# ctu-mrs/space_filling_forest_star

Hardware: AMD Instinct MI355X
Metric: accepted node expansions/sec + collision checks/sec, dense_3D 6-DoF (higher is better)
Workload: dtype f64

## Files before the change

space_filling_forest_star_amd/csrc/devforest.hip:

```cpp
#include <hip/hip_runtime.h>
#include <stdint.h>
#include <stdlib.h>
#include "kernels.h"
#include "sff_geom.h"
#include "kernels_dev.h"

namespace sffk {

using namespace sffg;

__device__ __forceinline__ int record_words_dev(int nbcap) { return 6 + 4 * nbcap; }

__device__ __forceinline__ int lemire_pick(unsigned long long word, unsigned long long range) {
  const unsigned long long lo = word * range;
  const unsigned long long hi = __umul64hi(word, range);
  if (lo < range) {
    const unsigned long long thr = (0ULL - range) % range;
    if (lo < thr) return -1;
  }
  return (int)hi;
}

__device__ __forceinline__ int32_t* frontier_now(const DevForestView& f) { return f.ctrl->front_sel ? f.frontier2 : f.frontier; }
__device__ __forceinline__ int32_t* act_now(const DevForestView& f) { return f.ctrl->act_sel ? f.act_slot2 : f.act_slot; }
// ... 159 lines not shown
#define KC_WLO 2
#define KC_WHI 3
#define KC_POSTED 4
#define KC_OWN 5
#define KC_CNT 6
#define KC_DEP 12
#define KC_EVN 13

__device__ __forceinline__ unsigned long long kc_load(const unsigned long long* p) {
  return __hip_atomic_load(p, __ATOMIC_RELAXED, __HIP_MEMORY_SCOPE_AGENT);
}
__device__ __forceinline__ void kc_publish(unsigned long long* p, unsigned seq, unsigned v) {
  __hip_atomic_store(p, ((unsigned long long)seq << 32) | (unsigned long long)v, __ATOMIC_RELAXED, __HIP_MEMORY_SCOPE_AGENT);
}
__device__ __forceinline__ unsigned kc_wait(const unsigned long long* p, unsigned seq, int32_t* fault) {
  for (int spin = 0; spin < KC_SPIN_LIMIT; ++spin) {
    const unsigned long long v = kc_load(p);
    if ((unsigned)(v >> 32) == seq) return (unsigned)v;
    __builtin_amdgcn_s_sleep(1);
  }
  atomicOr(fault, 1);
  return 0u;
}
__device__ __forceinline__ unsigned long long kc_block_sum(unsigned long long v, unsigned long long* slot) {
  for (int off = 32; off > 0; off >>= 1) v += __shfl_xor(v, off);
  __syncthreads();
  if (threadIdx.x == 0) *slot = 0ULL;
  __syncthreads();
  if ((threadIdx.x & 63) == 0 && v) atomicAdd(slot, v);
  __syncthreads();
  return *slot;
}

__device__ __forceinline__ void kc_block_sum8(unsigned long long* v, unsigned long long* slots, int from) {
  for (int q = from; q < 8; ++q)
    for (int off = 32; off > 0; off >>= 1) v[q] += __shfl_xor(v[q], off);
  __syncthreads();
  if (threadIdx.x < 8) slots[threadIdx.x] = 0ULL;
  __syncthreads();
  if ((threadIdx.x & 63) == 0)
    for (int q = from; q < 8; ++q) if (v[q]) atomicAdd(&slots[q], v[q]);
  __syncthreads();
  for (int q = from; q < 8; ++q) v[q] = slots[q];
}

__global__ __launch_bounds__(1024) void k_commit(ResolveArgs A, int n_bound) {
  __shared__ int s_state[64], s_dk[64], s_dep[64];
  __shared__ unsigned long long s_cnt[64][6];
  __shared__ unsigned long long s_sum;
  __shared__ unsigned long long s_wa, s_we, s_c6[7];
  __shared__ int s_ev_total;
  __shared__ unsigned long long s_tot[8];
  __shared__ DevCtrl K;
  const DevForestView& f = A.f;
  DevCtrl* c = f.ctrl;
  const int b = blockIdx.x;
  const int grp = threadIdx.x >> 4, gl = threadIdx.x & 15, lane = threadIdx.x & 63;
  const int i = b * 64 + grp;
  const bool inb = i < n_bound;
  const size_t s0 = (size_t)i * A.stride;
  const bool inl = inb && A.in_lim[i] != 0;
  const int flags = inb ? A.rec_flags[i] : 0;
  int nnb = inb ? A.rec_nnb[i] : 0;
  const bool pose_hit = inb && A.pose_hit[i] != 0;
  int fh = 0x7fffffff, ns = 0, nb = 0, meta = 0;
  if (inb) {
    fh = A.first_hit[s0 + gl]; ns = A.seg_ns[s0 + gl];
    if (gl > 0) { nb = A.rec_nb[(size_t)i * A.nbcap + gl - 1]; meta = A.rec_meta[(size_t)i * A.nbcap + gl - 1]; }
  }
  const int halt = c->halt, n = c->n_act;
  if (halt || n == 0) {
    if (b == 0 && threadIdx.x == 0) {
      c->app_n = 0;
      if (A.star) { A.S.hdr[0] = 0; A.S.hdr[1] = 1; A.S.hdr[2] = 0; A.S.hdr[4] = 0; }
    }
    return;
  }
  if (b == 0 && f.ord.hist)
    for (int r = threadIdx.x; r < f.ord.n_sub; r += 1024) (c->act_sel ? f.ord.cnt[0] : f.ord.cnt[1])[r * SFFK_ORD_CNT_STRIDE] = 0;
  if (b * 64 >= n) return;
  const int nwg = (n + 63) >> 6;
  const bool last = b == nwg - 1;
  const unsigned seq = (unsigned)f.commit_seq[0] + 1u;
  const int seq30 = (int)(seq & 0x3fffffffu);
  const int Tb = f.temp_base, N0 = c->N0, nb0 = c->n_borders;
  const unsigned long long stamp_hi = (c->epoch + 1ULL) << 32;
  unsigned long long* pub = f.wg_pub + (size_t)b * SFFK_PUB_WORDS;
  unsigned long long tk[6];
  const bool clk = last && f.profile;
  tk[0] = clk ? wall_clock64() : 0ULL;
  unsigned long long* trace = (f.kc_trace && (int)c->rounds == f.kc_trace_round && threadIdx.x == 0) ? f.kc_trace + 8 * (size_t)b : nullptr;
#define KC_TRACE(k) do { if (trace) trace[k] = wall_clock64(); } while (0)
  KC_TRACE(0);
  int work_items = 0;
  if (last) {
    for (int w = threadIdx.x; w < (int)(sizeof(DevCtrl) / 4); w += 1024)
      reinterpret_cast<int32_t*>(&K)[w] = reinterpret_cast<const int32_t*>(c)[w];
    work_items = A.round_ctrl[2];
  }

  auto calls_of = [](int fh, int ns) -> unsigned long long {
    return fh != 0x7fffffff ? (unsigned long long)fh : (unsigned long long)ns;
  };
  const int gsh = lane & 48;
  auto gballot = [&](bool p) -> unsigned { return (unsigned)((__ballot(p) >> gsh) & 0xffffULL); };
  auto gsum = [&](unsigned long long v) -> unsigned long long {
    for (int off = 8; off > 0; off >>= 1) v += __shfl_xor(v, off);
    return v;
  };
  unsigned long long cnt[6] = {0, 0, 0, 0, 0, 0};
  int st = 1, code = SFFK_REJECTED, dk = 0, was_dep = 0;
  const bool live = i < n;
  bool pending = false;
  if (nnb > 15) nnb = 15;
  const bool have = gl <= nnb;
  if (!have) { fh = 0x7fffffff; ns = 0; nb = 0; meta = 0; }
  const bool is_nb = have && gl > 0;
  const bool mate = is_nb && nb >= Tb;
  const bool same = (meta & 1) != 0;
  const bool fr = fh == 0x7fffffff;
  const unsigned long long my_calls = calls_of(fh, ns);
  const unsigned stops = gballot(is_nb && (mate || !same || fr));
  const unsigned mates = gballot(mate), sames = gballot(same), frees = gballot(fr);
  const bool goal_mode = f.goal_id >= 0;
  const unsigned goals = gballot(goal_mode && is_nb && nb == f.goal_id);
  bool count_end = true;
  if (live) {
    if (!inl) code = SFFK_OUTSIDE;
    else if (flags & 2) { if (gl == 0) { atomicOr(A.fault_pending, 1); atomicAdd(A.fault_pending + 1, 1); KC_FAULT_SETTLE(); } }
    else if ((flags & 3) == 1) {
      const bool ovf = gballot(have && fh == 0) != 0;
      const bool mine = A.world <= 1 || i % A.world == A.rank;
      const unsigned long long smp = gsum(have ? (unsigned long long)ns : 0ULL);
      if (mine) { cnt[3] = 1; cnt[4] = 1 + (unsigned long long)nnb; cnt[5] = smp; }
      const int fh0 = __shfl(fh, gsh), ns0 = __shfl(ns, gsh);
      if (ovf) { if (gl == 0) { atomicOr(A.fault_pending, 1); atomicAdd(A.fault_pending + 2, 1); KC_FAULT_SETTLE(); } }
      else {
        cnt[0] = 1;
        if (!pose_hit) {
          cnt[1] = 1;
          cnt[0] += calls_of(fh0, ns0);
          if (fh0 == 0x7fffffff) {
            cnt[2] = (unsigned long long)f.n_trees;
            pending = true;
          }
// ... 197 lines not shown
      ev_pref = (int)kc_block_sum(pe, &s_sum);
    }
    KC_TRACE(6);
    if (own) {
      const int at = nb0 + ev_pref + __popcll(wo & ((1ULL << threadIdx.x) - 1ULL));
      double pn[6], pe6[6], dn;
      int ta;
      const int raw = A.rec_nb[(size_t)e_i * A.nbcap + s_dk[threadIdx.x]];
      if (raw >= Tb) {
        const int j = raw - Tb;
        for (int q = 0; q < 6; ++q) pn[q] = A.newpos[6 * (size_t)j + q];
        dn = A.pdist[j] + f.d_root[A.parent[j]];
        ta = A.st.tree[A.parent[j]];
      } else {
        for (int q = 0; q < 6; ++q) pn[q] = A.st.pos[6 * (size_t)e_nb + q];
        dn = f.d_root[e_nb];
        ta = A.st.tree[e_nb];
      }
      const int tb = A.st.tree[e_ex];
      f.b_n1[at] = e_nb < e_ex ? e_nb : e_ex; f.b_n2[at] = e_nb < e_ex ? e_ex : e_nb;
      f.b_ta[at] = ta < tb ? ta : tb; f.b_tb[at] = ta < tb ? tb : ta;
      for (int q = 0; q < 6; ++q) pe6[q] = A.st.pos[6 * (size_t)e_ex + q];
      if (A.star) {
        const int e = at - nb0;
        A.S.ev_sample[e] = e_i; A.S.ev_nb[e] = e_nb; A.S.ev_ex[e] = e_ex; A.S.ev_dist[e] = dist6(pn, pe6);
        f.b_dist[at] = 0.0;
      } else
      f.b_dist[at] = dn + f.d_root[e_ex] + dist6(pn, pe6);
      f.pair[(size_t)ta * f.n_trees + tb] = 1;
      f.pair[(size_t)tb * f.n_trees + ta] = 1;
    }
  }
  KC_TRACE(7);
  if (!last) return;
  if (clk) tk[3] = wall_clock64();
  unsigned long long q_end = 0ULL, q_beg = ~0ULL;
  if (f.qclk_sh && threadIdx.x < 64) {
    q_end = f.qclk_sh[threadIdx.x * 16]; q_beg = f.qclk_sh[threadIdx.x * 16 + 1];
    for (int off = 32; off > 0; off >>= 1) {
      const unsigned long long e2 = __shfl_xor(q_end, off), b2 = __shfl_xor(q_beg, off);
      q_end = e2 > q_end ? e2 : q_end; q_beg = b2 < q_beg ? b2 : q_beg;
    }
  }
  unsigned long long tot[8] = {0, 0, 0, 0, 0, 0, 0, 0};
  if ((int)threadIdx.x < b) {
    const unsigned long long* pp = f.wg_pub + (size_t)threadIdx.x * SFFK_PUB_WORDS;
    for (int q = 0; q < 8; ++q) tot[q] = (unsigned)(early[q] >> 32) == seq ? (unsigned)early[q] : kc_wait(pp + KC_CNT + q, seq, f.commit_seq + 6);
  }
  if (threadIdx.x == 1023) s_ev_total = fault_seen;
  kc_block_sum8(tot, s_tot, 0);
  for (int q = 0; q < 7; ++q) tot[q] += s_c6[q];
  tot[7] += (unsigned long long)__popcll(we);
  const int n_acc = acc_pref + __popcll(wa), n_ev = defer ? (int)tot[7] : ev_pref + n_own, n_dep = (int)tot[6];
  const bool faulted = s_ev_total != 0;
  auto roll_back = [&](DevCtrl* k) {
    k->fault = SFFK_FAULT_LISTS;
    k->halt = 1;
    k->round -= 1;
    k->iter = k->iter0;
    k->cursor = k->words_base;
    k->rounds -= 1;
    k->round_nodes -= (unsigned long long)(k->N0 + n);
    k->round_queries -= (unsigned long long)n;
    k->n_act = 0;
    k->app_n = 0;
  };
  if (A.star && !faulted) {
    for (int w = threadIdx.x; w < (int)(sizeof(DevCtrl) / 4); w += 1024)
      reinterpret_cast<int32_t*>(A.S.backup)[w] = reinterpret_cast<const int32_t*>(&K)[w];
    __syncthreads();
    if (threadIdx.x == 0) roll_back(A.S.backup);
  }
  if (threadIdx.x == 0) {
    if (faulted) {
      roll_back(&K);
      *A.fault_pending = 0;
      if (A.star) { A.S.hdr[0] = 0; A.S.hdr[1] = 1; A.S.hdr[2] = 0; A.S.hdr[4] = 0; }
    } else {
      const int fn0 = K.frontier_n, act_cnt = K.act_cnt, act_sel = K.act_sel;
      K.collide_calls += tot[0];
      K.path_free_calls += tot[1];
      K.nn_queries += tot[2];
      K.poses_executed += tot[3];
      K.segments_executed += tot[4];
      K.samples_executed += tot[5];
      K.work_items += (unsigned long long)work_items;
      if (f.qclk_sh) { K.q_t0 = q_beg; K.q_t1 = q_end; }
      if (K.q_t1 > K.q_t0) { K.q_ticks += K.q_t1 - K.q_t0; K.q_launches += 1ULL; }
      K.app_n = n;
      K.app_N0 = N0;
      K.app_fn0 = fn0;
      K.app_act_sel = act_sel;
      K.app_act_cnt = act_cnt;
      K.iter0_app = K.iter0;
      K.n_nodes = N0 + n_acc;
      K.frontier_n = f.prio.n_heaps ? fn0 : fn0 + n_acc;
      K.n_borders = nb0 + n_ev;
      K.app_nb0 = nb0;
      K.n_unsettled += n_dep;
      K.epoch += 1ULL;
      if (A.star) {
        K.nn_queries += (unsigned long long)n_acc;
        A.S.hdr[0] = n_acc; A.S.hdr[1] = 0; A.S.hdr[2] = n_ev; A.S.hdr[3] = nb0; A.S.hdr[4] = 0;
      }
      K.act_sel = act_sel ^ 1;
      K.act_cnt = (n - n_acc) + (act_cnt - n);
      round_begin_scalars(f, &K);
      if (clk) {
        tk[4] = wall_clock64();
        for (int q = 0; q < 4; ++q) K.prof[q] += tk[q + 1] - tk[q];
      }
      K.prof[5] += (unsigned long long)passes;
      K.prof[6] += 1ULL;
      if ((unsigned long long)passes > K.prof[7]) K.prof[7] = (unsigned long long)passes;
    }
    f.commit_seq[0] = (int32_t)seq;
  }
  __syncthreads();
  for (int w = threadIdx.x; w < (int)(sizeof(DevCtrl) / 4); w += 1024)
    reinterpret_cast<int32_t*>(c)[w] = reinterpret_cast<const int32_t*>(&K)[w];
}

__device__ __forceinline__ void append_ord_store(const ResolveArgs& A, int ord_at, int next) {
  if (ord_at >= 0) (A.f.ctrl->app_act_sel ? A.f.ord.lst[0] : A.f.ord.lst[1])[ord_at] = next;
}
__device__ __forceinline__ int append_one(const ResolveArgs& A, int i, int& slot_out, int& ord_at, int part = 0) {
  ord_at = -1;
  const DevForestView& f = A.f;
  const DevCtrl* c = f.ctrl;
  const int n = c->app_n;
  slot_out = -1;
  if (n <= 0) return -1;
  const int act_cnt = c->app_act_cnt;
  const int32_t* act_old = c->app_act_sel ? f.act_slot2 : f.act_slot;
  int32_t* act_new = c->app_act_sel ? f.act_slot : f.act_slot2;
  const bool wave_over = c->n_act == 0 && !c->halt && c->in_wave && !c->use_closed;
  const bool ord_on = f.ord.hist && c->ord_valid;
  auto claim = [&](int e, int slot) {
    const int nd = f.slot_node[slot];
    atomicMin(&f.claim[nd], e);
    f.ulist[e] = nd;
  };
  if (wave_over && i == 0 && part != 1) f.ctrl->claims_done = 1;
  if (i >= n) {
    if (i < act_cnt && part != 1) {
      const int e = (c->act_cnt - (act_cnt - n)) + (i - n), slot = act_old[i];
      act_new[e] = slot;
      if (wave_over) claim(e, slot);
    }
    return -1;
  }
  const unsigned long long w = f.w_acc[i >> 6];
  const int rank = f.acc_pref[i >> 6] + __popcll(w & ((1ULL << (i & 63)) - 1ULL));
// ... 451 lines not shown
```

space_filling_forest_star_amd/csrc/engine.cpp:

```cpp
#include "engine.h"
#include <dlfcn.h>

#include <algorithm>
#include <chrono>
#include <cmath>
#include <cstdlib>
#include <cstring>
#include <limits>

#include "sff_geom.h"

namespace sff {

void hip_check(hipError_t e, const char* what) {
  if (e != hipSuccess) throw HipError{std::string(what) + ": " + hipGetErrorString(e)};
}
#define HIPCHK(x) hip_check((x), #x)

void DevBuf::ensure(size_t bytes) {
  if (bytes <= cap) return;
  size_t want = std::max(bytes, cap * 2);
  want = (want + 255) & ~(size_t)255;
  void* np = nullptr;
  HIPCHK(hipMalloc(&np, want));
// ... 262 lines not shown
  double ms = kernel_ms[kind];
  if (round_timed[kind]) ms += round_ms[kind] * ((double)round_calls[kind] / (double)round_timed[kind]);
  return ms;
}
void Ctx::sync() {
  HIPCHK(hipStreamSynchronize(stream));
  for (auto& t : pending) {
    float ms = 0;
    HIPCHK(hipEventElapsedTime(&ms, t.a, t.b));
    if (t.round) { round_ms[t.kind] += ms; round_timed[t.kind] += 1; }
    else kernel_ms[t.kind] += ms;
    kernel_launches[t.kind] += 1;
    pool.push_back(t.a);
    pool.push_back(t.b);
  }
  pending.clear();
}

static inline uint64_t spread21(uint64_t v) {
  v &= 0x1FFFFF;
  v = (v | v << 32) & 0x1F00000000FFFFULL;
  v = (v | v << 16) & 0x1F0000FF0000FFULL;
  v = (v | v << 8) & 0x100F00F00F00F00FULL;
  v = (v | v << 4) & 0x10C30C30C30C30C3ULL;
  v = (v | v << 2) & 0x1249249249249249ULL;
  return v;
}

void Ctx::upload_mesh(int role, const double* tri9, int n) {
  kn = Knobs::from_env();
  HIPCHK(hipSetDevice(device));
  if (role == SFFGPU_MESH_ROBOT) {
    if (n <= 0) throw HipError{"robot mesh must have at least one triangle"};
    rob_tri.ensure((size_t)n * 9 * sizeof(double));
    HIPCHK(hipMemcpy(rob_tri.p, tri9, (size_t)n * 9 * sizeof(double), hipMemcpyHostToDevice));
    robv.tri = rob_tri.as<double>();
    robv.n_tri = n;
    double lo[3] = {1e300, 1e300, 1e300}, hi[3] = {-1e300, -1e300, -1e300};
    for (int v = 0; v < n * 3; ++v)
      for (int i = 0; i < 3; ++i) {
        lo[i] = std::min(lo[i], tri9[3 * v + i]);
        hi[i] = std::max(hi[i], tri9[3 * v + i]);
      }
    double rad = 0;
    for (int i = 0; i < 3; ++i) { robv.lo[i] = lo[i]; robv.hi[i] = hi[i]; robv.center[i] = 0.5 * (lo[i] + hi[i]); }
    for (int v = 0; v < n * 3; ++v) {
      double d2 = 0;
      for (int i = 0; i < 3; ++i) d2 += (tri9[3 * v + i] - robv.center[i]) * (tri9[3 * v + i] - robv.center[i]);
      rad = std::max(rad, std::sqrt(d2));
    }
    robv.radius = rad;
    have_robot = true;
    h_rob.assign(tri9, tri9 + (size_t)n * 9);
    build_robot_extents();
    build_clearance();
    build_tri_grid();
    return;
  }
  if (role != SFFGPU_MESH_ENV) throw HipError{"unknown mesh role"};
  envv = sffk::EnvView{};
  have_env = true;
  clear_cells = 0;
  if (n <= 0) return;
  std::vector<double> box((size_t)n * 6);
  double glo[3] = {1e300, 1e300, 1e300}, ghi[3] = {-1e300, -1e300, -1e300};
  for (int t = 0; t < n; ++t)
    for (int a = 0; a < 3; ++a) {
      const double* P = tri9 + 9 * (size_t)t;
      double lo = std::min(P[a], std::min(P[3 + a], P[6 + a])), hi = std::max(P[a], std::max(P[3 + a], P[6 + a]));
// ... 1017 lines not shown
```

space_filling_forest_star_amd/csrc/forest_dev.cpp:

```cpp
#include <algorithm>
#include <chrono>
#include <cmath>
#include <cstdio>
#include <cstdlib>
#include <cstring>
#include <thread>
#include <vector>

#include "engine.h"
#include "sff_geom.h"

namespace sff {

#define HIPCHK(x) hip_check((x), #x)
using Clock = std::chrono::steady_clock;
static double ms_since(Clock::time_point t0) { return std::chrono::duration<double, std::milli>(Clock::now() - t0).count(); }

static uint64_t next_pow2(uint64_t v) {
  uint64_t p = 1;
  while (p < v) p <<= 1;
  return p;
}

bool Forest::device_eligible() const {
// ... 775 lines not shown
  c.r_items.ensure((size_t)B.list_cap * SFFK_ITEM_BYTES);
  c.r_sub.ensure((size_t)SFFK_SUBLISTS * SFFK_SUB_STRIDE * 4);
  return B;
}
static sffk::ResolveArgs dev_resolve_args(Forest& F, const DevRoundBufs& B) {
  Ctx& c = *F.ctx;
  DevEngine& d = F.dev;
  sffk::ResolveArgs ra{};
  ra.f = F.dev_view();
  ra.st = sffk::NodeStoreMut{c.sx.as<float>(), c.sy.as<float>(), c.sz.as<float>(), c.syaw.as<float>(),
                             c.spitch.as<float>(), c.sroll.as<float>(), c.stree.as<int32_t>(), c.spos.as<double>()};
  ra.g = c.gridv;
  ra.nbcap = B.NBCAP;
  ra.stride = B.STRIDE;
  ra.rank = F.cfg.rank;
  ra.world = F.cfg.world;
  ra.newpos = B.d_pos;
  ra.pdist = B.d_pd;
  ra.parent = (d.round_parity ? d.d_parent2 : d.d_parent).as<int32_t>();
  ra.code = B.code;
  ra.in_lim = B.d_lim;
  ra.rec_flags = B.d_rec;
  ra.pose_hit = B.d_pose;
  ra.rec_nnb = B.d_rec + B.n;
  ra.rec_nb = B.d_rec + 2 * (size_t)B.n;
  ra.rec_meta = B.d_rec + 2 * (size_t)B.n + (size_t)B.n * B.NBCAP;
  ra.seg_ns = B.seg_ns;
  ra.first_hit = B.first_hit;
  ra.bulk = B.bulk;
  ra.round_ctrl = B.d_rctrl;
  ra.fault_pending = d.fault_pending.as<int32_t>();
  ra.star = F.cfg.optimize ? 1 : 0;
  if (ra.star) ra.S = F.star_view();
  return ra;
}

size_t Forest::dev_exchange_bytes() const {
  const int per_rank = (cfg.wave + cfg.world - 1) / cfg.world;
  return (size_t)per_rank * sffk::record_words(kn.test_nbcap) * 4;
}

void Forest::dev_enqueue_begin() {
  Ctx& c = *ctx;
  DevEngine& d = dev;
  d.wr.wait_on(c.stream);
  sffk::launch_wave_begin(c.stream, dev_view());
}

static sffk::SampleLaunch dev_sample_launch(Forest& F, const DevRoundBufs& B) {
  Ctx& c = *F.ctx;
  DevEngine& d = F.dev;
  const sffk::DevForestView V = F.dev_view();
  sffk::NodeStoreMut stm{c.sx.as<float>(), c.sy.as<float>(), c.sz.as<float>(), c.syaw.as<float>(),
                         c.spitch.as<float>(), c.sroll.as<float>(), c.stree.as<int32_t>(), c.spos.as<double>()};
  sffk::SampleLaunch P{};
  memcpy(P.prm.limits, F.cfg.limits, sizeof P.prm.limits);
  P.prm.dist_tree = F.cfg.dist_tree;
  P.prm.sweep_abs_eps = c.sweep_eps();
  P.prm.rank = F.cfg.rank;
  P.prm.world = F.cfg.world;
  P.tmp.st = stm;
  P.tmp.cnt = c.r_cnt.as<int32_t>();
  P.tmp.tg = c.tgridv;
  P.tmp.ctrl = B.d_rctrl;
  P.tmp.sub = c.r_sub.as<int32_t>();
  P.tmp.n_perm = d.temp_base;
// ... 63 lines not shown
  ca.force = d.d_force.as<uint8_t>();
  ca.cnt = c.r_cnt.as<int32_t>();
  ca.hit_idx = nullptr;
  ca.hit_dist = nullptr;
  ca.tree = c.stree.as<int32_t>();
  ca.pos = c.spos.as<double>();
  ca.rec_flags = B.d_rec;
  ca.rec_nnb = ca.rec_flags + n;
  ca.rec_nb = ca.rec_nnb + n;
  ca.rec_meta = ca.rec_nb + (size_t)n * B.NBCAP;
  ca.seg_a = c.r_sega.as<double>();
  ca.seg_b = c.r_segb.as<double>();
  ca.seg_ns = B.seg_ns;
  ca.first_hit = B.first_hit;
  ca.seg_ovf = B.seg_ovf;
  ca.ctrl = B.d_rctrl;
  ca.dev_n = dev_n;
  ca.qclk = qclk;
  ca.qclk_sh = d.qclk_sh.as<unsigned long long>();
  if (V.ord.hist) {
    ca.ord_valid = reinterpret_cast<const int32_t*>(reinterpret_cast<char*>(d.ctrl.p) + offsetof(sffk::DevCtrl, ord_valid));
    ca.ord_nslots = reinterpret_cast<const int32_t*>(reinterpret_cast<char*>(d.ctrl.p) + offsetof(sffk::DevCtrl, n_slots));
    ca.ord_sel = reinterpret_cast<const int32_t*>(reinterpret_cast<char*>(d.ctrl.p) + offsetof(sffk::DevCtrl, act_sel));
    for (int q = 0; q < 2; ++q) { ca.ord_lst[q] = V.ord.lst[q]; ca.ord_cnt[q] = V.ord.cnt[q]; }
  }
  c.time_begin(T_SWEEP);
  ca.items = c.r_items.p;
  ca.items_cap = B.list_cap;
  ca.sub = c.r_sub.as<int32_t>();
  ca.pose_hit = B.d_pose;
  const bool blocked = sffk::launch_query_classify(c.stream, kn, c.gridv, &c.tgridv, c.store_view(), c.r_q.as<sffk::SweepQuery>(), ca, &c.envv);
  c.time_end();
  c.time_begin(T_COLLIDE);
  sffk::TempGridRef tref{c.tgridv, c.sx.as<float>() + d.temp_base, c.sy.as<float>() + d.temp_base,
                         c.sz.as<float>() + d.temp_base, n};
  sffk::TempGridRef tref_keep = tref;
  tref_keep.tg = sffk::GridView{};
  tref_keep.n = 0;
  sffk::launch_collide_items(c.stream, kn, c.envv, c.robv, B.d_pos, n, ca.rec_flags, B.d_pose, ca.seg_a, ca.seg_b, ca.seg_ns,
                             B.STRIDE, ca.ctrl, c.r_items.p, ca.items_cap, ca.sub, ca.first_hit, ca.seg_ovf,
                             cfg.optimize ? &tref_keep : &tref, dev_n, blocked ? &ca : nullptr);
  c.time_end();
  if (send_dev) {
    c.time_begin(T_EXCHANGE);
    sffk::launch_pack_records(c.stream, dev_resolve_args(*this, B), cfg.rank, cfg.world, n, static_cast<int32_t*>(send_dev));
    exchange_timer_drop();
    exchange_open = c.timed_now;
    if (exchange_open) { exchange_t = c.pending.back(); c.pending.pop_back(); }
  }
  c.timing_on = true;
  c.round_scope = false;
}

void Forest::dev_enqueue_round_commit(const void* recv_dev, bool sample_next) {
  Ctx& c = *ctx;
  const DevRoundBufs B = dev_round_bufs(*this);
  const sffk::ResolveArgs ra = dev_resolve_args(*this, B);
  if (recv_dev) {
    sffk::launch_unpack_records(c.stream, ra, cfg.rank, cfg.world, B.n, static_cast<const int32_t*>(recv_dev));
    if (exchange_open) {
      HIPCHK(hipEventRecord(exchange_t.b, c.stream));
      c.pending.push_back(exchange_t);
      exchange_open = false;
    }
  }
  sffk::SampleLaunch next{};
  if (sample_next) {
    dev.round_parity ^= 1;
    next = dev_sample_launch(*this, dev_round_bufs(*this));
    dev.round_parity ^= 1;
  }
  c.round_scope = true;
  c.timing_on = dev.round_timing;
  c.time_begin(T_COMMIT);
// ... 668 lines not shown
```

space_filling_forest_star_amd/csrc/kernels.h:

```cpp
#pragma once
#include <hip/hip_runtime.h>
#include <stdint.h>

#include "knobs.h"

namespace sffk {

struct NodeStoreView {
  const float* x;
  const float* y;
  const float* z;
  const float* yaw;
  const float* pitch;
  const float* roll;
  const int32_t* tree;
  const double* pos;
};

struct NodeStoreMut {
  float *x, *y, *z, *yaw, *pitch, *roll;
  int32_t* tree;
  double* pos;
};

// ... 58 lines not shown
#define SFFK_MAX_LEVELS 4
struct EnvView {
  const double* tri;
  const double* tri_box;
  const double* tri_plane;
  const double* tri_ext;
  const double* cand;
  int n_tri;
  int n_levels;
  const double* level_box[SFFK_MAX_LEVELS];
  int level_count[SFFK_MAX_LEVELS];
  const uint32_t* clear_bits;
  const uint32_t* clear_bits_edge;
  double clear_org[3];
  double clear_inv;
  int clear_n[3];
  const int32_t* tg_start;
  const int32_t* tg_list;
  double tg_org[3];
  double tg_inv;
  int tg_n[3];
};
void launch_tgrid_build(hipStream_t s, const EnvView& env, int32_t* cnt_or_start, int32_t* list, bool fill);
struct ClearBuildArgs {
  double thr_pose, thr_edge;
  double pose_lo[3], pose_hi[3];
  double edge_lo[3], edge_hi[3];
};
void launch_clear_build(hipStream_t s, const EnvView& env, const ClearBuildArgs& P, uint32_t* bits_pose, uint32_t* bits_edge,
                        long long n_cells);

struct RobotView {
  const double* tri;
  int n_tri;
  double center[3];
  double radius;
  double lo[3], hi[3];
};

struct DevCtrl {
  int32_t n_act;
  int32_t halt;
  int32_t n_nodes, iter, round, in_wave;
  int32_t n_slots, frontier_n, closed_n, use_closed;
  int32_t terminated, solved, empty_frontier, fault;
  int32_t N0, iter0, n_borders, n_unsettled;
  int32_t fault_pending, redraws, grid_ovf, tgrid_ovf;
  int32_t front_sel;
  int32_t compact_from;
  int32_t act_sel, act_cnt;
  int32_t app_n, app_N0, app_fn0, app_act_sel;
  int32_t iter0_app, app_act_cnt;
  int32_t claims_done;
  int32_t clear_n;
  unsigned long long cursor;
  unsigned long long words_base;
  unsigned long long collide_calls, path_free_calls, nn_queries;
  unsigned long long poses_executed, segments_executed, samples_executed;
  unsigned long long waves, rounds, round_nodes, round_queries;
  unsigned long long epoch;
  unsigned long long work_items;
  unsigned long long prof[8];
  unsigned long long q_t0, q_t1, q_ticks, q_launches;
  unsigned long long wprof[8];
  int32_t prio_n0, prio_wave, prio_all_empty, prio_gen;
  unsigned long long star_rounds, star_passes, star_members, star_rewires;
// ... 269 lines not shown
  double* best; int32_t* psel; double* dcl;
  unsigned long long* cnt;
  int32_t* acc_sample;
  int32_t* hdr;
  int32_t* changed;
  int32_t* ew; int32_t* ens; int32_t* first_hit; int32_t* seg_ovf; int32_t* ida; int32_t* idb;
  int32_t* sub;
  void* items; int items_cap;
  int32_t* ev_sample; int32_t* ev_nb; int32_t* ev_ex; double* ev_dist;
  unsigned long long* acc;
  DevCtrl* backup;
  unsigned long long* dbg;
  int32_t* hist; int32_t* hist_ctl; int hist_cap;
};
#define SFFK_DEPENDS 0
#define SFFK_REJECTED 1
#define SFFK_OUTSIDE 2
#define SFFK_ACCEPT 3
#define SFFK_REJECT_EVENT 4
struct ResolveArgs {
  DevForestView f;
  NodeStoreMut st;
  GridView g;
  int nbcap, stride;
  int rank, world;
  const double* newpos; const double* pdist; const int32_t* parent; uint8_t* code;
  const uint8_t* in_lim; int32_t* rec_flags; uint8_t* pose_hit;
  int32_t* rec_nnb; int32_t* rec_nb; int32_t* rec_meta; int32_t* seg_ns; int32_t* first_hit;
  unsigned long long* bulk;
  const int32_t* round_ctrl;
  int32_t* fault_pending;
  int star;
  StarView S;
};
void launch_wave_begin(hipStream_t s, const DevForestView& f);
void launch_prio_begin(hipStream_t s, const DevForestView& f);
void launch_prio_end(hipStream_t s, const DevForestView& f, const NodeStoreView& st);
void launch_prio_index(hipStream_t s, const PrioView& p);
struct SeqArgs {
  DevForestView f;
  NodeStoreMut st;
  GridView g;
  EnvView env;
  RobotView rob;
  double limits[6];
  double dist_tree, sampling_dist, sweep_abs_eps;
  const double* trig;
  unsigned long long words_end;
  int32_t* grid_ovf_src;
  int dim, max_waves, hit_cap, grid_ovf_limit;
  int optimize;
  const int32_t* ktab;
  int32_t* tree_cnt;
  int32_t* hist; int32_t* hist_ctl; int hist_cap;
  double cell_edge, knn_slack;
  int32_t* trace; int trace_cap;
};
void launch_seq_waves(hipStream_t s, const SeqArgs& a);
hipError_t launch_seq_waves_batch(hipStream_t s, const SeqArgs* members_dev, int n, bool optimize, bool priority, size_t lds);
#define SFFK_SPEC_DEPTH 4
#define SFFK_SPEC_TAB 20
#define SFFK_SPEC_REC 400
#define SFFK_SPEC_EARLY 384
struct SpecArgs {
  SeqArgs q;
  const int32_t* sc_tab;
// ... 92 lines not shown
```

space_filling_forest_star_amd/csrc/kernels.hip:

```cpp
#include <hip/hip_runtime.h>
#include <stdint.h>
#include <stdlib.h>
#include <string.h>
#include "kernels.h"
#include <algorithm>
#include "sff_geom.h"
#include "kernels_dev.h"
#include "star_pass_dev.h"
#include "prio_heap_dev.h"

namespace sffk {

using namespace sffg;


__global__ __launch_bounds__(256) void k_sample_steer(SampleLaunch P) {
  const int i = blockIdx.x * blockDim.x + threadIdx.x;
  sample_steer_one(i, P);
}

__device__ __forceinline__ float wrapf(float d) {
  const float PI_F = 3.14159274f;
  if (d < -PI_F) return d + 2.0f * PI_F;
  if (d >= PI_F) return d - 2.0f * PI_F;
// ... 3157 lines not shown
                                                                  int n_pose, const int32_t* __restrict__ live_flags,
                                                                  uint8_t* __restrict__ pose_hit,
                                                                  const double* __restrict__ a6, const double* __restrict__ b6,
                                                                  const int32_t* __restrict__ seg_ns, int stride,
                                                                  int32_t* __restrict__ ctrl,
                                                                  const SurvivorItem* __restrict__ list, int items_cap,
                                                                  const int32_t* __restrict__ sub,
                                                                  int32_t* __restrict__ first_hit,
                                                                  int32_t* __restrict__ overflow_flag, GridView tg,
                                                                  const float* __restrict__ tx, const float* __restrict__ ty,
                                                                  const float* __restrict__ tz, int n_temps,
                                                                  const int32_t* __restrict__ dev_n, TaskSource D) {
#ifdef SFFK_CI_TRACE
  const unsigned long long ci_entry = wall_clock64();
#endif
  if (dev_n) {
    if (dev_n[1]) return;
    n_pose = dev_n[0];
    if (n_temps) n_temps = dev_n[0];
  }
  extern __shared__ double lds_d[];
  double* rtri = lds_d;
  const int wave = threadIdx.x >> 6, lane = threadIdx.x & 63;
  int sub_n = sub[lane * SFFK_SUB_STRIDE], sub_nl = sub[lane * SFFK_SUB_STRIDE + 2];
  const int ctrl3 = ctrl[3];
  constexpr int CI_PRE = 6;
  const int n9 = rob.n_tri * 9;
  double rv[CI_PRE];
#pragma unroll
  for (int k = 0; k < CI_PRE; ++k) {
    const int idx = (int)threadIdx.x + k * 256;
    rv[k] = idx < n9 ? rob.tri[idx] : 0.0;
  }
  const int gt0 = blockIdx.x * blockDim.x + threadIdx.x;
  float cx0 = __int_as_float(0x7fc00000), cy0 = 0.0f, cz0 = 0.0f;
  if (tg.cnt && gt0 < n_temps) { cx0 = tx[gt0]; cy0 = ty[gt0]; cz0 = tz[gt0]; }
#pragma unroll
  for (int k = 0; k < CI_PRE; ++k) {
    const int idx = (int)threadIdx.x + k * 256;
    if (idx < n9) rtri[idx] = rv[k];
  }
  for (int i = (int)threadIdx.x + CI_PRE * 256; i < n9; i += blockDim.x) rtri[i] = rob.tri[i];
  if (tg.cnt) {
    if (cx0 == cx0) {
      const size_t cell = grid_cell_of(tg, cx0, cy0, cz0);
      tg.cnt[cell] = 0;
      if (tg.occ) tg.occ[cell >> 5] = 0u;
    }
    for (int t = gt0 + gridDim.x * blockDim.x; t < n_temps; t += gridDim.x * blockDim.x) {
      const float x = tx[t];
      if (x == x) {
        const size_t cell = grid_cell_of(tg, x, ty[t], tz[t]);
        tg.cnt[cell] = 0;
        if (tg.occ) tg.occ[cell >> 5] = 0u;
      }
    }
    if (blockIdx.x == 0 && threadIdx.x == 0) tg.ovf_cnt[0] = 0;
  }
  double* stage = rtri + (size_t)rob.n_tri * 9 + (size_t)wave * STAGE_DOUBLES;
  int32_t* ibase = reinterpret_cast<int32_t*>(rtri + (size_t)rob.n_tri * 9 + (size_t)SEG_WAVES * STAGE_DOUBLES);
  const int sub_cap = items_cap / SFFK_SUBLISTS, sub_half = sub_cap / 2;
  sub_n = sub_n < sub_half ? sub_n : sub_half;
  sub_nl = sub_nl < sub_cap - sub_half ? sub_nl : sub_cap - sub_half;
  int sub_incl = sub_n, sub_incl_l = sub_nl;
  for (int off = 1; off < 64; off <<= 1) {
    const int o = __shfl_up(sub_incl, off), ol = __shfl_up(sub_incl_l, off);
    if (lane >= off) { sub_incl += o; sub_incl_l += ol; }
  }
  const int MH = __shfl(sub_incl, 63);
  const int M = MH + __shfl(sub_incl_l, 63);
  const bool ran_over = ctrl3 != 0;
  if (blockIdx.x == 0 && threadIdx.x == 0) ctrl[2] = M;
  if ((M <= 0 && !ran_over) || env.n_tri == 0) return;
  __shared__ ShareArea s_share;
  share_init(s_share);
  __syncthreads();
  double* rbox = reinterpret_cast<double*>(ibase + SEG_WAVES * (STACK_CAP + TG_HASH + CAND_CAP + QUEUE_CAP));
  fill_robot_boxes(rtri, rbox, rob.n_tri, threadIdx.x, blockDim.x);
  __syncthreads();
  int32_t* stack = ibase + wave * (STACK_CAP + TG_HASH);
  int32_t* cand = ibase + SEG_WAVES * (STACK_CAP + TG_HASH) + wave * CAND_CAP;
  int32_t* queue = ibase + SEG_WAVES * (STACK_CAP + TG_HASH + CAND_CAP) + wave * QUEUE_CAP;
  DBG_DECL
  const int W = gridDim.x * SEG_WAVES;
#ifdef SFFK_CI_TRACE
  const unsigned long long ci_t0 = ci_entry, ci_pre = wall_clock64();
  const unsigned int ci_seen = __hip_atomic_load(&g_ci_launch, __ATOMIC_RELAXED, __HIP_MEMORY_SCOPE_AGENT);
  const bool ci_on = ci_seen == SFFK_CI_TRACE;
  int ci_items = 0;
  unsigned long long ci_first[4] = {0, 0, 0, 0};
#endif
  const int n_slots = n_pose * stride;
  const int E = ran_over ? n_pose + n_slots : M;
  int32_t* const ticket = const_cast<int32_t*>(sub) + (size_t)((blockIdx.x + gridDim.x * wave) & (SFFK_SUBLISTS - 1)) * SFFK_SUB_STRIDE + 1;
  auto next_item = [&](int e) -> int {
    if (ran_over) return e + W;
    int t = 0;
    if (lane == 0) t = atomicAdd(ticket, 1);
    t = __builtin_amdgcn_readfirstlane(t);
    return W + ((blockIdx.x + gridDim.x * wave) & (SFFK_SUBLISTS - 1)) + SFFK_SUBLISTS * t;
  };
  for (int e = blockIdx.x + gridDim.x * wave; e < E; e = next_item(e)) {
    int slot, c_lo, c_hi;
    unsigned long long mask = 0ULL;
    if (!ran_over) {
      size_t at;
      if (e < MH) {
        const int sl = __popcll(__ballot(sub_incl <= e));
        at = (size_t)sl * sub_cap + (e - (__shfl(sub_incl, sl) - __shfl(sub_n, sl)));
      } else {
        const int e2 = e - MH;
// ... 116 lines not shown
    const double* pb = store_pos + 6 * (size_t)sld<COH>(idb + slot);
    for (int k = 0; k < 6; ++k) { a[k] = pa[k]; b[k] = pb[k]; }
    segment_chunk(env, rob, E.rtri, E.rbox, E.stack, E.cand, E.queue, E.stage, a, b, slot, it.chunk, true, it.mask, first_hit,
                  overflow_flag, lane DBG_PASS, &s_share);
  }
  share_help(env, rob, E.rtri, E.rbox, E.queue, E.stage, E.cand_base, s_share, lane DBG_PASS);
}

__global__ __launch_bounds__(64 * SEG_WAVES) __attribute__((amdgpu_waves_per_eu(CI_OCC))) void k_star_exact(
    EnvView env, RobotView rob, const double* __restrict__ store_pos, const int32_t* __restrict__ ida,
    const int32_t* __restrict__ idb, const SurvivorItem* __restrict__ list, int items_cap, int32_t* __restrict__ sub,
    int32_t* __restrict__ first_hit, int32_t* __restrict__ overflow_flag, int32_t* __restrict__ hdr) {
  const int wave = threadIdx.x >> 6, lane = threadIdx.x & 63;
  int sub_n = sub[lane * SFFK_STAR_SUB];
  const int h_skip = hdr[1], h_fault = hdr[4];
  if (h_skip || h_fault) return;
  extern __shared__ double lds_d[];
  const ExactLds E = exact_lds(lds_d, rob.n_tri, wave);
  const int sub_cap = items_cap / SFFK_SUBLISTS;
  if (sub_n > sub_cap) {
    if (blockIdx.x == 0 && wave == 0) atomicOr(hdr + 4, 1);
    sub_n = sub_cap;
  }
  int sub_incl = sub_n;
  for (int off = 1; off < 64; off <<= 1) {
    const int o = __shfl_up(sub_incl, off);
    if (lane >= off) sub_incl += o;
  }
  const int M = __shfl(sub_incl, 63);
  if (M <= 0 || env.n_tri == 0) return;
  __shared__ ShareArea s_share;
  share_init(s_share);
  for (int i = threadIdx.x; i < rob.n_tri * 9; i += blockDim.x) E.rtri[i] = rob.tri[i];
  __syncthreads();
  fill_robot_boxes(E.rtri, E.rbox, rob.n_tri, threadIdx.x, blockDim.x);
  __syncthreads();
  star_exact_items<false>(env, rob, E, store_pos, ida, idb, list, sub_cap, sub, sub_n, sub_incl, M, first_hit, overflow_flag, s_share,
                          blockIdx.x, gridDim.x, wave, lane);
}

#define STAR_BAR_TICKS 4000000ULL
__device__ __forceinline__ void star_decide(int32_t* s_dec, const int32_t* fault, const int32_t* chg) {
  __syncthreads();
  if (threadIdx.x == 0) {
    s_dec[0] = __hip_atomic_load(fault, __ATOMIC_RELAXED, __HIP_MEMORY_SCOPE_AGENT);
    s_dec[1] = chg ? __hip_atomic_load(chg, __ATOMIC_RELAXED, __HIP_MEMORY_SCOPE_AGENT) : 0;
  }
  __syncthreads();
}
__device__ __forceinline__ void star_grid_barrier(int32_t* bar, int target, int32_t* fault, unsigned long long* dbg) {
  __builtin_amdgcn_fence(__ATOMIC_RELEASE, "workgroup");
  __builtin_amdgcn_s_waitcnt(0);
  __syncthreads();
  if (threadIdx.x == 0) {
    const unsigned long long ta = wall_clock64();
    __hip_atomic_fetch_add(bar, 1, __ATOMIC_RELAXED, __HIP_MEMORY_SCOPE_AGENT);
    const unsigned long long t0 = wall_clock64();
    while (__hip_atomic_load(bar, __ATOMIC_RELAXED, __HIP_MEMORY_SCOPE_AGENT) < target) {
      __builtin_amdgcn_s_sleep(2);
      if (wall_clock64() - t0 > STAR_BAR_TICKS) { atomicOr(fault, 1); break; }
    }
    const unsigned long long t1 = wall_clock64();
    if (dbg) { const unsigned long long t2 = wall_clock64(); dbg[0] += t0 - ta; dbg[1] += t1 - t0; dbg[2] += t2 - t1; }
  }
  __syncthreads();
}

__global__ __launch_bounds__(64 * SEG_WAVES) __attribute__((amdgpu_waves_per_eu(CI_OCC))) void k_star_tail(
// ... 33 lines not shown
  while (true) {
    const int slot = pass & (SFFK_STAR_PASSES - 1);
    if (wg == 0) {
      const int nx = (pass + 1) & (SFFK_STAR_PASSES - 1);
      for (int t = threadIdx.x; t < SFFK_SUBLISTS * SFFK_STAR_SUB; t += blockDim.x) sst<true>(S.sub + (size_t)nx * SFFK_SUBLISTS * SFFK_STAR_SUB + t, 0);
      if (threadIdx.x == 0) sst<true>(S.changed + nx, 0);
    }
    for (int r = wg * 4 + wave; r < h_n; r += g_act * 4)
      star_pass_sample<true>(A, env, st, slot, (r >> 2) & (SFFK_SUBLISTS - 1), S.acc_sample[r], N0, Tb, ep, L, wave, lane);
    if (dbg && threadIdx.x == 0) { const unsigned long long t = wall_clock64(); dbg[1] += 1; dbg[2] += t - tp; }
    star_grid_barrier(bar, ++n_bar * g_act, fault, dbg ? dbg + 4 : nullptr);
    if (dbg) tp = wall_clock64();
    star_decide(s_dec, fault, S.changed + slot);
    const int flt = s_dec[0], chg = s_dec[1];
    if (flt) break;
    if (chg == 0) { conv = true; break; }
    if (pass + 1 >= max_passes) break;
    int32_t* sub = S.sub + (size_t)slot * SFFK_SUBLISTS * SFFK_STAR_SUB;
    int sub_n = __hip_atomic_load(sub + lane * SFFK_STAR_SUB, __ATOMIC_RELAXED, __HIP_MEMORY_SCOPE_AGENT);
    const bool ran_over = __any(sub_n > sub_cap);
    if (ran_over) {
      if (wg == 0 && threadIdx.x == 0) atomicOr(fault, 1);
      break;
    }
    int sub_incl = sub_n;
    for (int off = 1; off < 64; off <<= 1) {
      const int o = __shfl_up(sub_incl, off);
      if (lane >= off) sub_incl += o;
    }
    const int M = __shfl(sub_incl, 63);
    if (M > 0 && env.n_tri != 0) {
      if (!robot_ready) {
        for (int i = threadIdx.x; i < rob.n_tri * 9; i += blockDim.x) E.rtri[i] = rob.tri[i];
        __syncthreads();
        fill_robot_boxes(E.rtri, E.rbox, rob.n_tri, threadIdx.x, blockDim.x);
        robot_ready = true;
      }
      share_init(s_share);
      __syncthreads();
      star_exact_items<true>(env, rob, E, st.pos, S.ida, S.idb, static_cast<const SurvivorItem*>(S.items), sub_cap, sub, sub_n, sub_incl,
                       M, S.first_hit, S.seg_ovf, s_share, wg, g_act, wave, lane);
    }
    if (M > 0) {
      if (dbg && threadIdx.x == 0) dbg[3] += wall_clock64() - tp;
      star_grid_barrier(bar, ++n_bar * g_act, fault, dbg ? dbg + 4 : nullptr);
      if (dbg) tp = wall_clock64();
      star_decide(s_dec, fault, nullptr);
      if (s_dec[0]) break;
    }
    ++pass;
  }
  if (conv)
    for (int e = wg * 256 + (int)threadIdx.x; e < n_ev; e += g_act * 256) star_pass_event<true>(f, S, e, ev_first, N0, ep);
  if (wg == 0 && threadIdx.x == 0) { S.hdr[STAR_PASSES_RUN] = pass + 1; S.hdr[STAR_CONVERGED] = conv ? 1 : 0; }
}

__global__ __launch_bounds__(256) void k_settle(SettleArgs A) {
  if (A.dev_n) {
    if (A.dev_n[1]) return;
    A.n = A.dev_n[0];
  }
  const int i = blockIdx.x * 256 + threadIdx.x;
  unsigned long long cc = 0, pf = 0, nq = 0, ns_settled = 0;
  unsigned long long ex_pose = 0, ex_seg = 0, ex_smp = 0;
  if (i < A.n) {
    int code = 0;
    if (!A.in_lim[i]) code = 2;
    else if (A.fault && (A.rec_flags[i] & 2)) atomicOr(A.fault, 1);
// ... 1937 lines not shown
```

Measured before the change: 11.34 million.

## Precompute robot boxes on host, move grid clear into commit, trim commit barriers

```diff
diff --git a/space_filling_forest_star_amd/csrc/devforest.hip b/space_filling_forest_star_amd/csrc/devforest.hip
--- a/space_filling_forest_star_amd/csrc/devforest.hip
+++ b/space_filling_forest_star_amd/csrc/devforest.hip
@@ -215,16 +215,10 @@
   return *slot;
 }
 
-__device__ __forceinline__ void kc_block_sum8(unsigned long long* v, unsigned long long* slots, int from) {
-  for (int q = from; q < 8; ++q)
-    for (int off = 32; off > 0; off >>= 1) v[q] += __shfl_xor(v[q], off);
-  __syncthreads();
-  if (threadIdx.x < 8) slots[threadIdx.x] = 0ULL;
-  __syncthreads();
-  if ((threadIdx.x & 63) == 0)
-    for (int q = from; q < 8; ++q) if (v[q]) atomicAdd(&slots[q], v[q]);
-  __syncthreads();
-  for (int q = from; q < 8; ++q) v[q] = slots[q];
+__device__ __forceinline__ void kc_wave_sync() {
+  __builtin_amdgcn_fence(__ATOMIC_RELEASE, "wavefront");
+  __builtin_amdgcn_wave_barrier();
+  __builtin_amdgcn_fence(__ATOMIC_ACQUIRE, "wavefront");
 }
 
 __global__ __launch_bounds__(1024) void k_commit(ResolveArgs A, int n_bound) {
@@ -233,8 +227,8 @@
   __shared__ unsigned long long s_sum;
   __shared__ unsigned long long s_wa, s_we, s_c6[7];
   __shared__ int s_ev_total;
-  __shared__ unsigned long long s_tot[8];
-  __shared__ DevCtrl K;
+  __shared__ unsigned long long s_part[16][8];
+  __shared__ DevCtrl K, KB;
   const DevForestView& f = A.f;
   DevCtrl* c = f.ctrl;
   const int b = blockIdx.x;
@@ -251,6 +245,8 @@
     fh = A.first_hit[s0 + gl]; ns = A.seg_ns[s0 + gl];
     if (gl > 0) { nb = A.rec_nb[(size_t)i * A.nbcap + gl - 1]; meta = A.rec_meta[(size_t)i * A.nbcap + gl - 1]; }
   }
+  float gx = __int_as_float(0x7fc00000), gy = 0.0f, gz = 0.0f;
+  if (A.clean.tg.cnt && inb && gl == 0) { gx = A.clean.x[i]; gy = A.clean.y[i]; gz = A.clean.z[i]; }
   const int halt = c->halt, n = c->n_act;
   if (halt || n == 0) {
     if (b == 0 && threadIdx.x == 0) {
@@ -276,10 +272,13 @@
 #define KC_TRACE(k) do { if (trace) trace[k] = wall_clock64(); } while (0)
   KC_TRACE(0);
   int work_items = 0;
+  unsigned long long q_end = 0ULL, q_beg = ~0ULL;
   if (last) {
+    if (f.qclk_sh && threadIdx.x < 64) { q_end = f.qclk_sh[threadIdx.x * 16]; q_beg = f.qclk_sh[threadIdx.x * 16 + 1]; }
     for (int w = threadIdx.x; w < (int)(sizeof(DevCtrl) / 4); w += 1024)
       reinterpret_cast<int32_t*>(&K)[w] = reinterpret_cast<const int32_t*>(c)[w];
     work_items = A.round_ctrl[2];
+    join_v(q_end, q_beg, work_items);
   }
 
   auto calls_of = [](int fh, int ns) -> unsigned long long {
@@ -294,6 +293,15 @@
   unsigned long long cnt[6] = {0, 0, 0, 0, 0, 0};
   int st = 1, code = SFFK_REJECTED, dk = 0, was_dep = 0;
   const bool live = i < n;
+  const int g_cell = (live && gx == gx) ? (int)grid_cell_of(A.clean.tg, gx, gy, gz) : -1;
+  auto clean_round_grid = [&]() {
+    if (!A.clean.tg.cnt) return;
+    if (g_cell >= 0) {
+      A.clean.tg.cnt[g_cell] = 0;
+      if (A.clean.tg.occ) A.clean.tg.occ[g_cell >> 5] = 0u;
+    }
+    if (b == 0 && threadIdx.x == 0) A.clean.tg.ovf_cnt[0] = 0;
+  };
   bool pending = false;
   if (nnb > 15) nnb = 15;
   const bool have = gl <= nnb;
@@ -557,27 +565,27 @@
     }
   }
   KC_TRACE(7);
-  if (!last) return;
+  if (!last) { clean_round_grid(); return; }
   if (clk) tk[3] = wall_clock64();
-  unsigned long long q_end = 0ULL, q_beg = ~0ULL;
-  if (f.qclk_sh && threadIdx.x < 64) {
-    q_end = f.qclk_sh[threadIdx.x * 16]; q_beg = f.qclk_sh[threadIdx.x * 16 + 1];
+  if (f.qclk_sh && threadIdx.x < 64)
     for (int off = 32; off > 0; off >>= 1) {
       const unsigned long long e2 = __shfl_xor(q_end, off), b2 = __shfl_xor(q_beg, off);
       q_end = e2 > q_end ? e2 : q_end; q_beg = b2 < q_beg ? b2 : q_beg;
     }
-  }
   unsigned long long tot[8] = {0, 0, 0, 0, 0, 0, 0, 0};
   if ((int)threadIdx.x < b) {
     const unsigned long long* pp = f.wg_pub + (size_t)threadIdx.x * SFFK_PUB_WORDS;
     for (int q = 0; q < 8; ++q) tot[q] = (unsigned)(early[q] >> 32) == seq ? (unsigned)early[q] : kc_wait(pp + KC_CNT + q, seq, f.commit_seq + 6);
   }
+  for (int q = 0; q < 8; ++q)
+    for (int off = 32; off > 0; off >>= 1) tot[q] += __shfl_xor(tot[q], off);
+  if (lane == 0)
+    for (int q = 0; q < 8; ++q) s_part[threadIdx.x >> 6][q] = tot[q];
   if (threadIdx.x == 1023) s_ev_total = fault_seen;
-  kc_block_sum8(tot, s_tot, 0);
-  for (int q = 0; q < 7; ++q) tot[q] += s_c6[q];
-  tot[7] += (unsigned long long)__popcll(we);
-  const int n_acc = acc_pref + __popcll(wa), n_ev = defer ? (int)tot[7] : ev_pref + n_own, n_dep = (int)tot[6];
+  __syncthreads();
+  clean_round_grid();
   const bool faulted = s_ev_total != 0;
+  if (threadIdx.x >= 64) return;
   auto roll_back = [&](DevCtrl* k) {
     k->fault = SFFK_FAULT_LISTS;
     k->halt = 1;
@@ -590,13 +598,19 @@
     k->n_act = 0;
     k->app_n = 0;
   };
-  if (A.star && !faulted) {
-    for (int w = threadIdx.x; w < (int)(sizeof(DevCtrl) / 4); w += 1024)
-      reinterpret_cast<int32_t*>(A.S.backup)[w] = reinterpret_cast<const int32_t*>(&K)[w];
-    __syncthreads();
-    if (threadIdx.x == 0) roll_back(A.S.backup);
+  const bool backup = A.star && !faulted;
+  if (backup) {
+    for (int w = threadIdx.x; w < (int)(sizeof(DevCtrl) / 4); w += 64)
+      reinterpret_cast<int32_t*>(&KB)[w] = reinterpret_cast<const int32_t*>(&K)[w];
+    kc_wave_sync();
   }
   if (threadIdx.x == 0) {
+    if (backup) roll_back(&KB);
+    for (int w = 1; w < 16; ++w)
+      for (int q = 0; q < 8; ++q) tot[q] += s_part[w][q];
+    for (int q = 0; q < 7; ++q) tot[q] += s_c6[q];
+    tot[7] += (unsigned long long)__popcll(we);
+    const int n_acc = acc_pref + __popcll(wa), n_ev = defer ? (int)tot[7] : ev_pref + n_own, n_dep = (int)tot[6];
     if (faulted) {
       roll_back(&K);
       *A.fault_pending = 0;
@@ -641,9 +655,11 @@
     }
     f.commit_seq[0] = (int32_t)seq;
   }
-  __syncthreads();
-  for (int w = threadIdx.x; w < (int)(sizeof(DevCtrl) / 4); w += 1024)
+  kc_wave_sync();
+  for (int w = threadIdx.x; w < (int)(sizeof(DevCtrl) / 4); w += 64) {
     reinterpret_cast<int32_t*>(c)[w] = reinterpret_cast<const int32_t*>(&K)[w];
+    if (backup) reinterpret_cast<int32_t*>(A.S.backup)[w] = reinterpret_cast<const int32_t*>(&KB)[w];
+  }
 }
 
 __device__ __forceinline__ void append_ord_store(const ResolveArgs& A, int ord_at, int next) {
diff --git a/space_filling_forest_star_amd/csrc/engine.cpp b/space_filling_forest_star_amd/csrc/engine.cpp
--- a/space_filling_forest_star_amd/csrc/engine.cpp
+++ b/space_filling_forest_star_amd/csrc/engine.cpp
@@ -318,9 +318,17 @@
   HIPCHK(hipSetDevice(device));
   if (role == SFFGPU_MESH_ROBOT) {
     if (n <= 0) throw HipError{"robot mesh must have at least one triangle"};
-    rob_tri.ensure((size_t)n * 9 * sizeof(double));
+    std::vector<double> h_box((size_t)n * 6);
+    for (int r = 0; r < n; ++r)
+      for (int ax = 0; ax < 3; ++ax) {
+        h_box[6 * (size_t)r + ax] = sffg::min3(tri9[9 * (size_t)r + ax], tri9[9 * (size_t)r + 3 + ax], tri9[9 * (size_t)r + 6 + ax]);
+        h_box[6 * (size_t)r + 3 + ax] = sffg::max3(tri9[9 * (size_t)r + ax], tri9[9 * (size_t)r + 3 + ax], tri9[9 * (size_t)r + 6 + ax]);
+      }
+    rob_tri.ensure((size_t)n * 15 * sizeof(double));
     HIPCHK(hipMemcpy(rob_tri.p, tri9, (size_t)n * 9 * sizeof(double), hipMemcpyHostToDevice));
+    HIPCHK(hipMemcpy(rob_tri.as<double>() + (size_t)n * 9, h_box.data(), (size_t)n * 6 * sizeof(double), hipMemcpyHostToDevice));
     robv.tri = rob_tri.as<double>();
+    robv.box = robv.tri + (size_t)n * 9;
     robv.n_tri = n;
     double lo[3] = {1e300, 1e300, 1e300}, hi[3] = {-1e300, -1e300, -1e300};
     for (int v = 0; v < n * 3; ++v)
diff --git a/space_filling_forest_star_amd/csrc/forest_dev.cpp b/space_filling_forest_star_amd/csrc/forest_dev.cpp
--- a/space_filling_forest_star_amd/csrc/forest_dev.cpp
+++ b/space_filling_forest_star_amd/csrc/forest_dev.cpp
@@ -831,6 +831,9 @@
   ra.fault_pending = d.fault_pending.as<int32_t>();
   ra.star = F.cfg.optimize ? 1 : 0;
   if (ra.star) ra.S = F.star_view();
+  else
+    ra.clean = sffk::TempGridRef{c.tgridv, c.sx.as<float>() + d.temp_base, c.sy.as<float>() + d.temp_base,
+                                 c.sz.as<float>() + d.temp_base, B.n};
   return ra;
 }
 
@@ -960,14 +963,9 @@
   const bool blocked = sffk::launch_query_classify(c.stream, kn, c.gridv, &c.tgridv, c.store_view(), c.r_q.as<sffk::SweepQuery>(), ca, &c.envv);
   c.time_end();
   c.time_begin(T_COLLIDE);
-  sffk::TempGridRef tref{c.tgridv, c.sx.as<float>() + d.temp_base, c.sy.as<float>() + d.temp_base,
-                         c.sz.as<float>() + d.temp_base, n};
-  sffk::TempGridRef tref_keep = tref;
-  tref_keep.tg = sffk::GridView{};
-  tref_keep.n = 0;
   sffk::launch_collide_items(c.stream, kn, c.envv, c.robv, B.d_pos, n, ca.rec_flags, B.d_pose, ca.seg_a, ca.seg_b, ca.seg_ns,
                              B.STRIDE, ca.ctrl, c.r_items.p, ca.items_cap, ca.sub, ca.first_hit, ca.seg_ovf,
-                             cfg.optimize ? &tref_keep : &tref, dev_n, blocked ? &ca : nullptr);
+                             nullptr, dev_n, blocked ? &ca : nullptr);
   c.time_end();
   if (send_dev) {
     c.time_begin(T_EXCHANGE);
diff --git a/space_filling_forest_star_amd/csrc/kernels.h b/space_filling_forest_star_amd/csrc/kernels.h
--- a/space_filling_forest_star_amd/csrc/kernels.h
+++ b/space_filling_forest_star_amd/csrc/kernels.h
@@ -114,6 +114,7 @@
 
 struct RobotView {
   const double* tri;
+  const double* box;
   int n_tri;
   double center[3];
   double radius;
@@ -449,6 +450,7 @@
   int32_t* fault_pending;
   int star;
   StarView S;
+  TempGridRef clean;
 };
 void launch_wave_begin(hipStream_t s, const DevForestView& f);
 void launch_prio_begin(hipStream_t s, const DevForestView& f);
diff --git a/space_filling_forest_star_amd/csrc/kernels.hip b/space_filling_forest_star_amd/csrc/kernels.hip
--- a/space_filling_forest_star_amd/csrc/kernels.hip
+++ b/space_filling_forest_star_amd/csrc/kernels.hip
@@ -3213,6 +3213,14 @@
     const int idx = (int)threadIdx.x + k * 256;
     rv[k] = idx < n9 ? rob.tri[idx] : 0.0;
   }
+  constexpr int CI_PRE_BOX = 4;
+  const int n6 = rob.n_tri * 6;
+  double rbv[CI_PRE_BOX];
+#pragma unroll
+  for (int k = 0; k < CI_PRE_BOX; ++k) {
+    const int idx = (int)threadIdx.x + k * 256;
+    rbv[k] = idx < n6 ? rob.box[idx] : 0.0;
+  }
   const int gt0 = blockIdx.x * blockDim.x + threadIdx.x;
   float cx0 = __int_as_float(0x7fc00000), cy0 = 0.0f, cz0 = 0.0f;
   if (tg.cnt && gt0 < n_temps) { cx0 = tx[gt0]; cy0 = ty[gt0]; cz0 = tz[gt0]; }
@@ -3222,6 +3230,15 @@
     if (idx < n9) rtri[idx] = rv[k];
   }
   for (int i = (int)threadIdx.x + CI_PRE * 256; i < n9; i += blockDim.x) rtri[i] = rob.tri[i];
+  double* stage = rtri + (size_t)rob.n_tri * 9 + (size_t)wave * STAGE_DOUBLES;
+  int32_t* ibase = reinterpret_cast<int32_t*>(rtri + (size_t)rob.n_tri * 9 + (size_t)SEG_WAVES * STAGE_DOUBLES);
+  double* rbox = reinterpret_cast<double*>(ibase + SEG_WAVES * (STACK_CAP + TG_HASH + CAND_CAP + QUEUE_CAP));
+#pragma unroll
+  for (int k = 0; k < CI_PRE_BOX; ++k) {
+    const int idx = (int)threadIdx.x + k * 256;
+    if (idx < n6) rbox[idx] = rbv[k];
+  }
+  for (int i = (int)threadIdx.x + CI_PRE_BOX * 256; i < n6; i += blockDim.x) rbox[i] = rob.box[i];
   if (tg.cnt) {
     if (cx0 == cx0) {
       const size_t cell = grid_cell_of(tg, cx0, cy0, cz0);
@@ -3238,8 +3255,6 @@
     }
     if (blockIdx.x == 0 && threadIdx.x == 0) tg.ovf_cnt[0] = 0;
   }
-  double* stage = rtri + (size_t)rob.n_tri * 9 + (size_t)wave * STAGE_DOUBLES;
-  int32_t* ibase = reinterpret_cast<int32_t*>(rtri + (size_t)rob.n_tri * 9 + (size_t)SEG_WAVES * STAGE_DOUBLES);
   const int sub_cap = items_cap / SFFK_SUBLISTS, sub_half = sub_cap / 2;
   sub_n = sub_n < sub_half ? sub_n : sub_half;
   sub_nl = sub_nl < sub_cap - sub_half ? sub_nl : sub_cap - sub_half;
@@ -3255,9 +3270,6 @@
   if ((M <= 0 && !ran_over) || env.n_tri == 0) return;
   __shared__ ShareArea s_share;
   share_init(s_share);
-  __syncthreads();
-  double* rbox = reinterpret_cast<double*>(ibase + SEG_WAVES * (STACK_CAP + TG_HASH + CAND_CAP + QUEUE_CAP));
-  fill_robot_boxes(rtri, rbox, rob.n_tri, threadIdx.x, blockDim.x);
   __syncthreads();
   int32_t* stack = ibase + wave * (STACK_CAP + TG_HASH);
   int32_t* cand = ibase + SEG_WAVES * (STACK_CAP + TG_HASH) + wave * CAND_CAP;
@@ -3440,8 +3452,7 @@
   __shared__ ShareArea s_share;
   share_init(s_share);
   for (int i = threadIdx.x; i < rob.n_tri * 9; i += blockDim.x) E.rtri[i] = rob.tri[i];
-  __syncthreads();
-  fill_robot_boxes(E.rtri, E.rbox, rob.n_tri, threadIdx.x, blockDim.x);
+  for (int i = threadIdx.x; i < rob.n_tri * 6; i += blockDim.x) E.rbox[i] = rob.box[i];
   __syncthreads();
   star_exact_items<false>(env, rob, E, store_pos, ida, idb, list, sub_cap, sub, sub_n, sub_incl, M, first_hit, overflow_flag, s_share,
                           blockIdx.x, gridDim.x, wave, lane);
@@ -3541,8 +3552,7 @@
     if (M > 0 && env.n_tri != 0) {
       if (!robot_ready) {
         for (int i = threadIdx.x; i < rob.n_tri * 9; i += blockDim.x) E.rtri[i] = rob.tri[i];
-        __syncthreads();
-        fill_robot_boxes(E.rtri, E.rbox, rob.n_tri, threadIdx.x, blockDim.x);
+        for (int i = threadIdx.x; i < rob.n_tri * 6; i += blockDim.x) E.rbox[i] = rob.box[i];
         robot_ready = true;
       }
       share_init(s_share);
```

New measurement: 11.30 million. Within noise of the previous version (-0.4%).
